# microsoft/Spartan

Measured on AMD Instinct MI355X. Metric: R1CS constraints/sec in SNARK::prove (synthetic 2^20); bit-exact proof, higher is better.
Workload: dtype u64x4 (F_q Montgomery / F_p 2^255-19 limbs)

## Files before the change

spartan_amd/csrc/fe10.hpp:

```cpp
#pragma once
#include "field.hpp"

namespace sp {

struct Fe10 {
  int32_t v[10];
};

SP_HD void fe10_pin(Fe10& a) {
#if defined(__HIP_DEVICE_COMPILE__)
#pragma unroll
  for (int i = 0; i < 10; i++) asm volatile("" : "+v"(a.v[i]));
#else
  (void)a;
#endif
}

SP_HD Fe10 fe10_from_fp(const Fp& x) {
  Fp c = fp_canon(x);
  const int off[10] = {0, 26, 51, 77, 102, 128, 153, 179, 204, 230};
  Fe10 r;
#pragma unroll
  for (int i = 0; i < 10; i++) {
    int w = off[i] >> 6, s = off[i] & 63, bits = (i & 1) ? 25 : 26;
    uint64_t lo = c.v[w] >> s;
    if (s + bits > 64 && w < 3) lo |= c.v[w + 1] << (64 - s);
    r.v[i] = (int32_t)(lo & (((uint64_t)1 << bits) - 1));
  }
  return r;
}
SP_HD Fp fe10_to_fp(const Fe10& a) {
  int32_t h[10];
#pragma unroll
  for (int i = 0; i < 10; i++) h[i] = a.v[i];
  int32_t q = (19 * h[9] + (1 << 24)) >> 25;
#pragma unroll
  for (int i = 0; i < 10; i++) q = (h[i] + q) >> ((i & 1) ? 25 : 26);
  h[0] += 19 * q;
#pragma unroll
  for (int i = 0; i < 9; i++) {
    int sh = (i & 1) ? 25 : 26;
    int32_t c = h[i] >> sh;
    h[i + 1] += c;
    h[i] -= c << sh;
  }
  h[9] -= (h[9] >> 25) << 25;
  const int off[10] = {0, 26, 51, 77, 102, 128, 153, 179, 204, 230};
  Fp r = fp_zero();
#pragma unroll
  for (int i = 0; i < 10; i++) {
    int w = off[i] >> 6, s = off[i] & 63;
    uint64_t x = (uint64_t)(uint32_t)h[i];
    r.v[w] |= x << s;
    if (s > 38 && w < 3) r.v[w + 1] |= x >> (64 - s);
  }
  return r;
}

SP_HD Fe10 fe10_add(const Fe10& a, const Fe10& b) {
  Fe10 r;
#pragma unroll
  for (int i = 0; i < 10; i++) r.v[i] = a.v[i] + b.v[i];
  return r;
}
SP_HD Fe10 fe10_sub(const Fe10& a, const Fe10& b) {
  Fe10 r;
#pragma unroll
  for (int i = 0; i < 10; i++) r.v[i] = a.v[i] - b.v[i];
  return r;
}
SP_HD Fe10 fe10_neg(const Fe10& a) {
  Fe10 r;
#pragma unroll
  for (int i = 0; i < 10; i++) r.v[i] = -a.v[i];
  return r;
}
SP_HD Fe10 fe10_select(const Fe10& a, const Fe10& b, bool take_b) {
  Fe10 r;
#pragma unroll
  for (int i = 0; i < 10; i++) r.v[i] = take_b ? b.v[i] : a.v[i];
  return r;
}
SP_HD Fe10 fe10_one() { return Fe10{{1, 0, 0, 0, 0, 0, 0, 0, 0, 0}}; }

SP_HD Fe10 fe10_carry(int64_t h[10]) {
  int64_t c;
  c = (h[0] + (1 << 25)) >> 26; h[1] += c; h[0] -= c << 26;
  c = (h[4] + (1 << 25)) >> 26; h[5] += c; h[4] -= c << 26;
  c = (h[1] + (1 << 24)) >> 25; h[2] += c; h[1] -= c << 25;
  c = (h[5] + (1 << 24)) >> 25; h[6] += c; h[5] -= c << 25;
  c = (h[2] + (1 << 25)) >> 26; h[3] += c; h[2] -= c << 26;
  c = (h[6] + (1 << 25)) >> 26; h[7] += c; h[6] -= c << 26;
  c = (h[3] + (1 << 24)) >> 25; h[4] += c; h[3] -= c << 25;
  c = (h[7] + (1 << 24)) >> 25; h[8] += c; h[7] -= c << 25;
  c = (h[4] + (1 << 25)) >> 26; h[5] += c; h[4] -= c << 26;
  c = (h[8] + (1 << 25)) >> 26; h[9] += c; h[8] -= c << 26;
  c = (h[9] + (1 << 24)) >> 25; h[0] += c * 19; h[9] -= c << 25;
  c = (h[0] + (1 << 25)) >> 26; h[1] += c; h[0] -= c << 26;
  Fe10 r;
#pragma unroll
  for (int i = 0; i < 10; i++) r.v[i] = (int32_t)h[i];
  return r;
}
SP_HD Fe10 fe10_load(const Fp& x) {
  Fe10 t = fe10_from_fp(x);
  int64_t h[10];
#pragma unroll
  for (int i = 0; i < 10; i++) h[i] = t.v[i];
  return fe10_carry(h);
}
SP_HD Fe10 fe10_mul(const Fe10& f, const Fe10& g) {
  int32_t g19[10], f2[10];
#pragma unroll
  for (int i = 0; i < 10; i++) {
    g19[i] = 19 * g.v[i];
    f2[i] = 2 * f.v[i];
  }
  int64_t h[10];
#pragma unroll
  for (int k = 0; k < 10; k++) h[k] = 0;
#pragma unroll
  for (int i = 0; i < 10; i++)
#pragma unroll
    for (int j = 0; j < 10; j++) {
      int32_t a = ((i & 1) && (j & 1)) ? f2[i] : f.v[i];
      int32_t b = (i + j >= 10) ? g19[j] : g.v[j];
      h[(i + j) % 10] += (int64_t)a * b;
    }
  return fe10_carry(h);
}
SP_HD Fe10 fe10_sqr(const Fe10& f) {
  int32_t f19[10], f2[10];
#pragma unroll
  for (int i = 0; i < 10; i++) {
    f19[i] = 19 * f.v[i];
    f2[i] = 2 * f.v[i];
  }
  int64_t h[10];
#pragma unroll
  for (int k = 0; k < 10; k++) h[k] = 0;
#pragma unroll
  for (int i = 0; i < 10; i++) {
    {
      int32_t a = (i & 1) ? f2[i] : f.v[i];
      int32_t b = (2 * i >= 10) ? f19[i] : f.v[i];
      h[(2 * i) % 10] += (int64_t)a * b;
    }
#pragma unroll
    for (int j = i + 1; j < 10; j++) {
      int32_t a = f2[i];
      int32_t b = (i + j >= 10) ? f19[j] : f.v[j];
      int64_t prod = (int64_t)a * b;
      h[(i + j) % 10] += ((i & 1) && (j & 1)) ? 2 * prod : prod;
    }
  }
  return fe10_carry(h);
}
SP_HD Fe10 fe10_pow2k(Fe10 a, int k) {
  for (int i = 0; i < k; i++) a = fe10_sqr(a);
  return a;
}
SP_HD void fe10_pow_ladder(const Fe10& z, Fe10* z2_250_0, Fe10* z11) {
  Fe10 z2 = fe10_sqr(z);
  Fe10 z9 = fe10_mul(fe10_pow2k(z2, 2), z);
  *z11 = fe10_mul(z9, z2);
  Fe10 z2_5_0 = fe10_mul(fe10_sqr(*z11), z9);
  Fe10 z2_10_0 = fe10_mul(fe10_pow2k(z2_5_0, 5), z2_5_0);
  Fe10 z2_20_0 = fe10_mul(fe10_pow2k(z2_10_0, 10), z2_10_0);
  Fe10 z2_40_0 = fe10_mul(fe10_pow2k(z2_20_0, 20), z2_20_0);
  Fe10 z2_50_0 = fe10_mul(fe10_pow2k(z2_40_0, 10), z2_10_0);
  Fe10 z2_100_0 = fe10_mul(fe10_pow2k(z2_50_0, 50), z2_50_0);
  Fe10 z2_200_0 = fe10_mul(fe10_pow2k(z2_100_0, 100), z2_100_0);
  *z2_250_0 = fe10_mul(fe10_pow2k(z2_200_0, 50), z2_50_0);
}
SP_HD Fe10 fe10_pow_p58(const Fe10& x) {
  Fe10 t, z11;
  fe10_pow_ladder(x, &t, &z11);
  return fe10_mul(fe10_pow2k(t, 2), x);
}
SP_HD Fp fp_pow_p58_serial(const Fp& z) {
  Fe10 x = fe10_load(z);
  fe10_pin(x);
  return fe10_to_fp(fe10_pow_p58(x));
}
SP_HD Fp fp_invert_serial(const Fp& z) {
  Fe10 x = fe10_load(z);
  fe10_pin(x);
  Fe10 t, z11;
  fe10_pow_ladder(x, &t, &z11);
  return fe10_to_fp(fe10_mul(fe10_pow2k(t, 5), z11));
}

}
```

spartan_amd/csrc/tree.hpp:

```cpp
#pragma once
#include "curve.hpp"

__device__ __forceinline__ Fe10 fe10_pick(const Fe10& a, const Fe10& b, bool take_b) { return fe10_select(a, b, take_b); }
__device__ __forceinline__ void tree_wave_handover() {
  __builtin_amdgcn_fence(__ATOMIC_RELEASE, "wavefront");
  __builtin_amdgcn_wave_barrier();
  __builtin_amdgcn_fence(__ATOMIC_ACQUIRE, "wavefront");
}
__device__ __forceinline__ Fe10 fe10_quad_perm_1032(const Fe10& a) {
  Fe10 r;
#pragma unroll
  for (int i = 0; i < 10; i++) r.v[i] = __builtin_amdgcn_mov_dpp(a.v[i], 0xB1 , 0xF, 0xF, true);
  return r;
}
__device__ __forceinline__ Fe10 fe10_quad_perm_1302(const Fe10& a) {
  Fe10 r;
#pragma unroll
  for (int i = 0; i < 10; i++) r.v[i] = __builtin_amdgcn_mov_dpp(a.v[i], 0x8D , 0xF, 0xF, true);
  return r;
}
__device__ __forceinline__ void pt10_tree_quad(Pt10* sm, Fe10* , size_t n) {
  const int t = threadIdx.x, role = t & 3;
  const Fe10 zero = Fe10{{0, 0, 0, 0, 0, 0, 0, 0, 0, 0}};
  const Fe10 k2d = fe10_pick(fe10_one(), fe10_load(fp_D2()), role == 2);
  const int fsel = role <= 1 ? 1 : (role == 2 ? 3 : 2);
  const int gsel = role <= 1 ? 0 : (role == 2 ? 3 : 2);
  const int osel = role == 0 ? 3 : (role == 1 ? 1 : (role == 2 ? 0 : 2));
  int top = 128;
  while (top > 1 && (size_t)top >= n) top >>= 1;
  for (int s = top; s > 0; s >>= 1) {
    for (int base = 0; base < s; base += 64) {
      const int q = base + (t >> 2);
      const bool act = q < s && (size_t)(q + s) < n;
      if (act) {
        Fe10* P = reinterpret_cast<Fe10*>(sm + q);
        const Fe10* Q = reinterpret_cast<const Fe10*>(sm + q + s);
        Fe10 f1 = P[fsel], g1 = P[gsel], f2 = Q[fsel], g2 = Q[gsel];
        g1 = fe10_pick(g1, fe10_neg(g1), role == 0);
        g1 = fe10_pick(g1, zero, role == 2);
        g2 = fe10_pick(g2, fe10_neg(g2), role == 0);
        g2 = fe10_pick(g2, zero, role >= 2);
        Fe10 u = fe10_add(f1, g1), v = fe10_add(f2, g2);
        Fe10 mine = fe10_mul(u, fe10_mul(v, k2d));
        Fe10 other = fe10_quad_perm_1032(mine);
        Fe10 val = (role & 1) ? fe10_add(mine, other) : fe10_sub(other, mine);
        Fe10 fac = fe10_quad_perm_1302(val);
        P[osel] = fe10_mul(val, fac);
      }
    }
    if (s > 16) __syncthreads();
    else tree_wave_handover();
  }
  __syncthreads();
}
__device__ __forceinline__ void pt10_tree_quad_ded(Pt10* sm, unsigned char* idf, size_t n) {
  const int t = threadIdx.x, role = t & 3;
  const Fe10 zero = Fe10{{0, 0, 0, 0, 0, 0, 0, 0, 0, 0}};
  const int fP = role <= 1 ? 1 : role;
  const int gP = role <= 1 ? 0 : role;
  const int fQ = role <= 1 ? 1 : (role == 2 ? 3 : 2);
  const int osel = role == 0 ? 2 : (role == 1 ? 1 : (role == 2 ? 0 : 3));
  int top = 128;
  while (top > 1 && (size_t)top >= n) top >>= 1;
  for (int s = top; s > 0; s >>= 1) {
    for (int base = 0; base < s; base += 64) {
      const int q = base + (t >> 2);
      const bool act = q < s && (size_t)(q + s) < n;
      if (act) {
        Fe10* P = reinterpret_cast<Fe10*>(sm + q);
        const Fe10* Q = reinterpret_cast<const Fe10*>(sm + q + s);
        const bool idP = idf[q] != 0, idQ = idf[q + s] != 0;
        if (!idQ) {
          if (idP) {
            P[role] = Q[role];
            if (role == 0) idf[q] = 0;
          } else {
            Fe10 f1 = P[fP], g1 = P[gP], f2 = Q[fQ], g2 = Q[0];
            g1 = fe10_pick(g1, fe10_neg(g1), role == 0);
            g2 = fe10_pick(fe10_pick(g2, fe10_neg(g2), role == 1), zero, role >= 2);
            Fe10 mine = fe10_mul(fe10_add(f1, g1), fe10_add(f2, g2));
            Fe10 other = fe10_quad_perm_1032(mine);
            Fe10 minuend = fe10_pick(mine, other, role == 0), subtrahend = fe10_pick(other, mine, role == 0);
            Fe10 val = (role == 1 || role == 2) ? fe10_add(mine, other) : fe10_sub(minuend, subtrahend);
            Fe10 fac = fe10_quad_perm_1302(val);
            P[osel] = fe10_mul(val, fac);
          }
        }
      }
    }
    if (s > 16) __syncthreads();
    else tree_wave_handover();
  }
  __syncthreads();
}
__device__ __forceinline__ bool pt10_is_blank(const Pt10& p) {
  int32_t acc = 0;
#pragma unroll
  for (int i = 0; i < 10; i++) acc |= p.X.v[i] | p.T.v[i];
#pragma unroll
  for (int i = 1; i < 10; i++) acc |= p.Y.v[i] | p.Z.v[i];
  return acc == 0 && p.Y.v[0] == 1 && p.Z.v[0] == 1;
}
```

Baseline: 46.83 million.

## Spread field multiplies across 16 lanes per coordinate in the last tree levels

For the final reduction levels (s<=4) of the point-addition trees, each field multiply is split so every lane computes one output limb. Operand forms go through a shared exchange buffer, and carries pass between neighbouring lanes via ds_bpermute. This targets the tail levels, where only a few quads are active and most of the wave sits idle. The cost is extra LDS traffic, wave barriers, a parallel carry scheme, and __syncthreads at more levels.

```diff
diff --git a/spartan_amd/csrc/fe10.hpp b/spartan_amd/csrc/fe10.hpp
--- a/spartan_amd/csrc/fe10.hpp
+++ b/spartan_amd/csrc/fe10.hpp
@@ -102,6 +102,77 @@
   for (int i = 0; i < 10; i++) r.v[i] = (int32_t)h[i];
   return r;
 }
+struct Fe10Forms {
+  int32_t f[10], fd[10], w[20];
+};
+SP_HD void fe10_forms_first(Fe10Forms& o, int i, int32_t v) {
+  o.f[i] = v;
+  o.fd[i] = (i & 1) ? 2 * v : v;
+}
+SP_HD void fe10_forms_second(Fe10Forms& o, int i, int32_t v) {
+  o.w[i] = 19 * v;
+  o.w[10 + i] = v;
+}
+SP_HD int64_t fe10_sum_from_forms(const int32_t* fa, const int32_t* w, int k) {
+  int64_t h = 0;
+#pragma unroll
+  for (int i = 0; i < 10; i++) h += (int64_t)fa[i] * w[10 + k - i];
+  return h;
+}
+SP_HD int64_t fe10_mul_sum(const Fe10Forms& first, const Fe10Forms& second, int k) {
+  return fe10_sum_from_forms((k & 1) ? first.f : first.fd, second.w, k);
+}
+SP_HD int64_t fe10_sqr_sum(const Fe10& f, int k) {
+  int64_t h = 0;
+#pragma unroll
+  for (int i = 0; i < 10; i++) {
+    const int j = (k - i + 10) % 10;
+    if (j < i) continue;
+    const int32_t b = (i + j >= 10) ? 19 * f.v[j] : f.v[j];
+    if (j == i) h += (int64_t)((i & 1) ? 2 * f.v[i] : f.v[i]) * b;
+    else {
+      const int64_t prod = (int64_t)(2 * f.v[i]) * b;
+      h += ((i & 1) && (j & 1)) ? 2 * prod : prod;
+    }
+  }
+  return h;
+}
+SP_HD void fe10_lane_span(int lanes, int lane, int* lo, int* hi) {
+  const int per = (10 + lanes - 1) / lanes;
+  const int a = lane * per, b = a + per;
+  *lo = a < 10 ? a : 10;
+  *hi = b < 10 ? b : 10;
+}
+SP_HD void fe10_mul_share(const Fe10& f, const Fe10& g, int lanes, int lane, int64_t h[10]) {
+  Fe10Forms ff, gf;
+  for (int i = 0; i < 10; i++) {
+    fe10_forms_first(ff, i, f.v[i]);
+    fe10_forms_second(gf, i, g.v[i]);
+  }
+  int lo, hi;
+  fe10_lane_span(lanes, lane, &lo, &hi);
+  for (int k = lo; k < hi; k++) h[k] = fe10_mul_sum(ff, gf, k);
+}
+SP_HD void fe10_sqr_share(const Fe10& f, int lanes, int lane, int64_t h[10]) {
+  int lo, hi;
+  fe10_lane_span(lanes, lane, &lo, &hi);
+  for (int k = lo; k < hi; k++) h[k] = fe10_sqr_sum(f, k);
+}
+SP_HD int64_t fe10_carry_out(int64_t h, int k) { return (k & 1) ? (h + (1 << 24)) >> 25 : (h + (1 << 25)) >> 26; }
+SP_HD int64_t fe10_carry_split(int64_t h, int k, int64_t* c) {
+  *c = fe10_carry_out(h, k);
+  return h - *c * ((int64_t)1 << ((k & 1) ? 25 : 26));
+}
+SP_HD int64_t fe10_carry_in(int64_t c_below, int k) { return k == 0 ? 19 * c_below : c_below; }
+SP_HD Fe10 fe10_carry_par(const int64_t h[10]) {
+  int64_t r[10], c[10];
+  for (int k = 0; k < 10; k++) r[k] = fe10_carry_split(h[k], k, &c[k]);
+  for (int k = 0; k < 10; k++) r[k] += fe10_carry_in(c[(k + 9) % 10], k);
+  for (int k = 0; k < 10; k++) r[k] = fe10_carry_split(r[k], k, &c[k]);
+  Fe10 out;
+  for (int k = 0; k < 10; k++) out.v[k] = (int32_t)(r[k] + fe10_carry_in(c[(k + 9) % 10], k));
+  return out;
+}
 SP_HD Fe10 fe10_load(const Fp& x) {
   Fe10 t = fe10_from_fp(x);
   int64_t h[10];
diff --git a/spartan_amd/csrc/tree.hpp b/spartan_amd/csrc/tree.hpp
--- a/spartan_amd/csrc/tree.hpp
+++ b/spartan_amd/csrc/tree.hpp
@@ -19,7 +19,107 @@
   for (int i = 0; i < 10; i++) r.v[i] = __builtin_amdgcn_mov_dpp(a.v[i], 0x8D , 0xF, 0xF, true);
   return r;
 }
-__device__ __forceinline__ void pt10_tree_quad(Pt10* sm, Fe10* , size_t n) {
+#if defined(SP_TREE_QUAD_ONLY)
+#define SP_TREE_WIDE_MAX 0
+#else
+#define SP_TREE_WIDE_MAX 4
+#endif
+struct WideSlot {
+  Fe10Forms op;
+};
+static_assert(16 * sizeof(WideSlot) + 256 <= 256 * sizeof(Fe10), "the wide levels' slots share the exchange buffer with the 256 marks of the dedicated tree");
+__device__ __forceinline__ int32_t wide_lane_get(int32_t v, int src_lane) { return __builtin_amdgcn_ds_bpermute(src_lane << 2, v); }
+__device__ __forceinline__ int32_t wide_carry(int64_t h, int k, int below) {
+  int64_t c;
+  int64_t r = fe10_carry_split(h, k, &c);
+  const int32_t chi = wide_lane_get((int32_t)(c >> 32), below), clo = wide_lane_get((int32_t)c, below);
+  r += fe10_carry_in(((int64_t)chi << 32) | (uint32_t)clo, k);
+  r = fe10_carry_split(r, k, &c);
+  return (int32_t)(r + fe10_carry_in((int64_t)wide_lane_get((int32_t)c, below), k));
+}
+__device__ __forceinline__ int32_t wide_mul_limb(const WideSlot* fs, const WideSlot* ws, int k, bool live, int below) {
+  int64_t h = 0;
+  if (live) h = fe10_sum_from_forms((k & 1) ? fs->op.f : fs->op.fd, ws->op.w, k);
+  return wide_carry(h, k, below);
+}
+__device__ __forceinline__ int32_t wide_second_product(WideSlot* slots, int32_t mine, int k, bool live, int below, bool add, bool neg_mine) {
+  const int sl = threadIdx.x >> 4, role = sl & 3;
+  WideSlot* own = slots + sl;
+  const int32_t other = wide_lane_get(mine, (threadIdx.x & 63) ^ 16);
+  const int32_t val = add ? mine + other : (neg_mine ? other - mine : mine - other);
+  if (live) {
+    fe10_forms_first(own->op, k, val);
+    fe10_forms_second(own->op, k, val);
+  }
+  tree_wave_handover();
+  const int src = role == 0 ? 1 : (role == 1 ? 3 : (role == 2 ? 0 : 2));
+  return wide_mul_limb(own, slots + (sl & ~3) + src, k, live, below);
+}
+__device__ __forceinline__ void pt10_wide_level(Pt10* sm, WideSlot* slots, int s, size_t n, int32_t k2d_limb) {
+  const int t = threadIdx.x, q = t >> 6, sl = t >> 4, role = sl & 3, k = t & 15;
+  if (!(q < s && (size_t)(q + s) < n)) return;
+  const bool live = k < 10;
+  const int below = (t & 63) + (k == 0 ? 9 : -1);
+  const int fsel = role <= 1 ? 1 : (role == 2 ? 3 : 2);
+  const int gsel = role <= 1 ? 0 : (role == 2 ? 3 : 2);
+  const int osel = role == 0 ? 3 : (role == 1 ? 1 : (role == 2 ? 0 : 2));
+  Fe10* P = reinterpret_cast<Fe10*>(sm + q);
+  const Fe10* Q = reinterpret_cast<const Fe10*>(sm + q + s);
+  WideSlot* own = slots + sl;
+  int32_t u = 0;
+  if (live) {
+    int32_t g1 = P[gsel].v[k], g2 = Q[gsel].v[k];
+    g1 = role == 0 ? -g1 : (role == 2 ? 0 : g1);
+    g2 = role == 0 ? -g2 : (role >= 2 ? 0 : g2);
+    u = P[fsel].v[k] + g1;
+    fe10_forms_first(own->op, k, Q[fsel].v[k] + g2);
+    fe10_forms_second(own->op, k, k2d_limb);
+  }
+  tree_wave_handover();
+  const int32_t v2 = wide_mul_limb(own, own, k, live, below);
+  if (live) {
+    fe10_forms_first(own->op, k, u);
+    fe10_forms_second(own->op, k, v2);
+  }
+  tree_wave_handover();
+  const int32_t mine = wide_mul_limb(own, own, k, live, below);
+  const int32_t out = wide_second_product(slots, mine, k, live, below, (role & 1) != 0, true);
+  if (live) P[osel].v[k] = out;
+}
+__device__ __forceinline__ void pt10_wide_level_ded(Pt10* sm, unsigned char* idf, WideSlot* slots, int s, size_t n) {
+  const int t = threadIdx.x, q = t >> 6, sl = t >> 4, role = sl & 3, k = t & 15;
+  if (!(q < s && (size_t)(q + s) < n)) return;
+  const bool idP = idf[q] != 0, idQ = idf[q + s] != 0;
+  if (idQ) return;
+  tree_wave_handover();
+  if (idP) {
+    const int l = t & 63;
+    if (l < 40) reinterpret_cast<int32_t*>(sm + q)[l] = reinterpret_cast<const int32_t*>(sm + q + s)[l];
+    if (l == 0) idf[q] = 0;
+    return;
+  }
+  const bool live = k < 10;
+  const int below = (t & 63) + (k == 0 ? 9 : -1);
+  const int fP = role <= 1 ? 1 : role;
+  const int gP = role <= 1 ? 0 : role;
+  const int fQ = role <= 1 ? 1 : (role == 2 ? 3 : 2);
+  const int osel = role == 0 ? 2 : (role == 1 ? 1 : (role == 2 ? 0 : 3));
+  Fe10* P = reinterpret_cast<Fe10*>(sm + q);
+  const Fe10* Q = reinterpret_cast<const Fe10*>(sm + q + s);
+  WideSlot* own = slots + sl;
+  if (live) {
+    int32_t g1 = P[gP].v[k], g2 = Q[0].v[k];
+    g1 = role == 0 ? -g1 : g1;
+    g2 = role == 1 ? -g2 : (role >= 2 ? 0 : g2);
+    fe10_forms_first(own->op, k, P[fP].v[k] + g1);
+    fe10_forms_second(own->op, k, Q[fQ].v[k] + g2);
+  }
+  tree_wave_handover();
+  const int32_t mine = wide_mul_limb(own, own, k, live, below);
+  const int32_t out = wide_second_product(slots, mine, k, live, below, role == 1 || role == 2, role == 0);
+  if (live) P[osel].v[k] = out;
+}
+__device__ __forceinline__ void pt10_tree_quad(Pt10* sm, Fe10* xch, size_t n) {
   const int t = threadIdx.x, role = t & 3;
   const Fe10 zero = Fe10{{0, 0, 0, 0, 0, 0, 0, 0, 0, 0}};
   const Fe10 k2d = fe10_pick(fe10_one(), fe10_load(fp_D2()), role == 2);
@@ -28,7 +128,26 @@
   const int osel = role == 0 ? 3 : (role == 1 ? 1 : (role == 2 ? 0 : 2));
   int top = 128;
   while (top > 1 && (size_t)top >= n) top >>= 1;
+#if SP_TREE_WIDE_MAX > 0
+  WideSlot* const slots = reinterpret_cast<WideSlot*>(xch);
+  const Fe10 d2 = fe10_load(fp_D2());
+  int32_t k2d_limb = (t & 15) == 0 ? 1 : 0;
+  if (((t >> 4) & 3) == 2) {
+#pragma unroll
+    for (int i = 0; i < 10; i++) k2d_limb = (t & 15) == i ? d2.v[i] : k2d_limb;
+    if ((t & 15) >= 10) k2d_limb = 0;
+  }
+#else
+  (void)xch;
+#endif
   for (int s = top; s > 0; s >>= 1) {
+#if SP_TREE_WIDE_MAX > 0
+    if (s <= SP_TREE_WIDE_MAX) {
+      pt10_wide_level(sm, slots, s, n, k2d_limb);
+      __syncthreads();
+      continue;
+    }
+#endif
     for (int base = 0; base < s; base += 64) {
       const int q = base + (t >> 2);
       const bool act = q < s && (size_t)(q + s) < n;
@@ -48,7 +167,7 @@
         P[osel] = fe10_mul(val, fac);
       }
     }
-    if (s > 16) __syncthreads();
+    if (s > 16 || s <= 2 * SP_TREE_WIDE_MAX) __syncthreads();
     else tree_wave_handover();
   }
   __syncthreads();
@@ -63,6 +182,13 @@
   int top = 128;
   while (top > 1 && (size_t)top >= n) top >>= 1;
   for (int s = top; s > 0; s >>= 1) {
+#if SP_TREE_WIDE_MAX > 0
+    if (s <= SP_TREE_WIDE_MAX) {
+      pt10_wide_level_ded(sm, idf, reinterpret_cast<WideSlot*>(idf + 256), s, n);
+      __syncthreads();
+      continue;
+    }
+#endif
     for (int base = 0; base < s; base += 64) {
       const int q = base + (t >> 2);
       const bool act = q < s && (size_t)(q + s) < n;
@@ -88,7 +214,7 @@
         }
       }
     }
-    if (s > 16) __syncthreads();
+    if (s > 16 || s <= 2 * SP_TREE_WIDE_MAX) __syncthreads();
     else tree_wave_handover();
   }
   __syncthreads();
```

New measurement: 47.70 million, median of 6. 1.9% higher.
